# joybio/multiPrime

Measured on AMD Instinct MI355X. Metric: candidate x sequence coverage evals/s, higher is better.
Workload: dtype u32; 1 GPU; synthetic MSA 1048576 x 1000, k=18, v=1, 8 candidates/window, 950 windows, strict -c 2,3,-1 per GPU x 1 GPU(s) = BASELINE configs[3] itself (SURVEY 8d input 4; synthetic 1M x 1 kb; shape 1x1: row shards x window groups); rows_per_gpu=1048576, rows_total=1048576, cols=1000, k=18, variation=1, candidates_per_window=8, windows=950, parallelism=one GPU holds every row

## Files before the change

### multiprime_amd/csrc/evalslide.hip

```cpp
#include "common.hpp"
#include "bitslice.hpp"
#include "slidecore.hpp"
#include "evalslide.hpp"
#include "chainbody.hpp"

using namespace mp;

namespace {

typedef unsigned int u32x4 __attribute__((ext_vector_type(4)));
typedef unsigned int u32x2 __attribute__((ext_vector_type(2)));

struct SlideKernArgs {
    SlideArgs A;
    const uint32_t *cols32;
    const uint32_t *excl32;
    int nw32;
    unsigned long long *out;
    int wc, wc_pad;
    int max_items;
    int n_slide_blocks;
    EvalChainArgs chain;
    unsigned long long *clear;
    uint32_t n_clear;
    int patch_words;
    unsigned long long *stamps;
};

template <int GW>
struct DevEnv {
    const SlideKernArgs &K;
    __amdgpu_buffer_rsrc_t rs_cols, rs_excl;
    int voff, lane;
    uint32_t row_bytes;
    bool live;
    uint32_t *ring;
    uint32_t *tab;
    uint32_t itv;
    uint32_t live_mask;

    __device__ __forceinline__ DevEnv(const SlideKernArgs &k) : K(k) {}
    __device__ __forceinline__ void progress(int quarter) const {
#ifndef SLIDE_NO_PRIO
        if (quarter <= 0) __builtin_amdgcn_s_setprio(3);
        else if (quarter == 1) __builtin_amdgcn_s_setprio(2);
        else if (quarter == 2) __builtin_amdgcn_s_setprio(1);
        else __builtin_amdgcn_s_setprio(0);
#endif
    }
    __device__ __forceinline__ void stamp(int i) const {
        if (K.stamps && threadIdx.x == 0) K.stamps[(size_t)blockIdx.x * 8 + i] = wall_clock64();
    }
    __device__ __forceinline__ SlideBand uband(int b) const {
        const SlideBand *p = K.A.bands + b;
        SlideBand r;
        r.w0 = __builtin_amdgcn_readfirstlane(p->w0); r.n_win = __builtin_amdgcn_readfirstlane(p->n_win);
        r.item0 = __builtin_amdgcn_readfirstlane(p->item0); r.n_items = __builtin_amdgcn_readfirstlane(p->n_items);
        r.iter0 = __builtin_amdgcn_readfirstlane(p->iter0); r.pad = 0;
        return r;
    }
    __device__ __forceinline__ void load_iters(int idx) { itv = K.A.iters[(size_t)idx + (size_t)lane]; }
    __device__ __forceinline__ uint32_t iter_word(int j) const { return (uint32_t)__builtin_amdgcn_readlane((int)itv, j); }
    typedef const uint32_t __attribute__((address_space(4))) * ConstWords;
    struct Rec { uint32_t w[8], sm_lo, sm_hi, flags; ConstWords p; };
    __device__ __forceinline__ Rec load_rec(int item) const {
        Rec r;
        r.p = (ConstWords)(K.A.recs + (size_t)__builtin_amdgcn_readfirstlane(item) * kSlideRec);
#pragma unroll
        for (int q = 0; q < 8; q++) r.w[q] = r.p[q];
        r.sm_lo = r.p[24]; r.sm_hi = r.p[25]; r.flags = r.p[28];
        return r;
    }
    __device__ __forceinline__ uint32_t rec_word(const Rec &r, int q) const {
        return q < 8 ? r.w[q] : (q == 24 ? r.sm_lo : (q == 25 ? r.sm_hi : (q == 28 ? r.flags : r.p[q])));
    }
    __device__ __forceinline__ uint32_t rec_word_dyn(const Rec &r, int q) const { return r.p[q]; }
    template <int AUX = 0>
    __device__ __forceinline__ void load(__amdgpu_buffer_rsrc_t rs, int soff, uint32_t (&d)[GW]) const {
        if constexpr (GW == 4) {
            const u32x4 v = __builtin_amdgcn_raw_buffer_load_b128(rs, voff, soff, AUX);
            d[0] = v.x; d[1] = v.y; d[2] = v.z; d[3] = v.w;
        } else if constexpr (GW == 2) {
            const u32x2 v = __builtin_amdgcn_raw_buffer_load_b64(rs, voff, soff, AUX);
            d[0] = v.x; d[1] = v.y;
        } else {
            d[0] = __builtin_amdgcn_raw_buffer_load_b32(rs, voff, soff, AUX);
        }
    }
#ifndef SLIDE_EXP_ONE_ROW
#define SLIDE_EXP_ONE_ROW 0
#endif
#ifndef SLIDE_COL_AUX
#define SLIDE_COL_AUX 2
#endif
#ifndef SLIDE_EVT_AUX
#define SLIDE_EVT_AUX 0
#endif
    __device__ __forceinline__ void fetch(uint32_t row_off, uint32_t (&d)[GW]) const {
        load<SLIDE_COL_AUX>(rs_cols, SLIDE_EXP_ONE_ROW == 1 || SLIDE_EXP_ONE_ROW == 3 ? 0 : (int)row_off, d);
    }
    __device__ __forceinline__ void fetch_event(uint32_t row_off, uint32_t (&d)[GW]) const {
        load<SLIDE_EVT_AUX>(rs_cols, SLIDE_EXP_ONE_ROW == 1 || SLIDE_EXP_ONE_ROW == 2 ? 0 : (int)row_off, d);
    }
    __device__ __forceinline__ void valid_of(uint32_t row_off, uint32_t (&v)[GW]) const {
        load(rs_excl, (int)row_off, v);
#pragma unroll
        for (int i = 0; i < GW; i++) v[i] = bop<kSlAndNot>(live_mask, v[i], 0u);
    }
    __device__ __forceinline__ void ring_put(uint32_t *p, const uint32_t (&v)[GW]) const {
        if constexpr (GW == 4) *reinterpret_cast<u32x4 *>(p) = u32x4{v[0], v[1], v[2], v[3]};
        else if constexpr (GW == 2) *reinterpret_cast<u32x2 *>(p) = u32x2{v[0], v[1]};
        else p[0] = v[0];
    }
    __device__ __forceinline__ void ring_get(const uint32_t *p, uint32_t (&v)[GW]) const {
        if constexpr (GW == 4) { const u32x4 t = *reinterpret_cast<const u32x4 *>(p); v[0] = t.x; v[1] = t.y; v[2] = t.z; v[3] = t.w; }
        else if constexpr (GW == 2) { const u32x2 t = *reinterpret_cast<const u32x2 *>(p); v[0] = t.x; v[1] = t.y; }
        else v[0] = p[0];
    }
    __device__ __forceinline__ void ring_zero(int k) {
        uint32_t z[GW];
#pragma unroll
        for (int i = 0; i < GW; i++) z[i] = 0u;
        for (int s = 0; s < k; s++) ring_put(ring + s * (64 * GW), z);
    }
    __device__ __forceinline__ void ring_write(int slot, const uint32_t (&in)[GW]) { ring_put(ring + slot * (64 * GW), in); }
    __device__ __forceinline__ void ring_read(int slot, uint32_t (&o)[GW]) const { ring_get(ring + slot * (64 * GW), o); }
    __device__ __forceinline__ void commit(int idx, const uint32_t (&accPF)[8], const uint32_t (&accR)[4]) {
        uint32_t x0 = accPF[0], x1 = accPF[1], x2 = accPF[2], x3 = accPF[3], x4 = accPF[4], x5 = accPF[5], x6 = accPF[6], x7 = accPF[7];
        uint32_t x8 = accR[0], x9 = accR[1], x10 = accR[2], x11 = accR[3];
        asm volatile(
            "s_nop 1\n\t"
            "v_add_u32_dpp %0, %0, %0 row_ror:4 row_mask:0xf bank_mask:0x5\n\t"
            "v_add_u32_dpp %2, %2, %2 row_ror:4 row_mask:0xf bank_mask:0x5\n\t"
            "v_add_u32_dpp %4, %4, %4 row_ror:4 row_mask:0xf bank_mask:0x5\n\t"
            "v_add_u32_dpp %6, %6, %6 row_ror:4 row_mask:0xf bank_mask:0x5\n\t"
            "v_add_u32_dpp %8, %8, %8 row_ror:4 row_mask:0xf bank_mask:0x5\n\t"
            "v_add_u32_dpp %10, %10, %10 row_ror:4 row_mask:0xf bank_mask:0x5\n\t"
            "v_add_u32_dpp %0, %1, %1 row_ror:4 row_mask:0xf bank_mask:0xa\n\t"
            "v_add_u32_dpp %2, %3, %3 row_ror:4 row_mask:0xf bank_mask:0xa\n\t"
            "v_add_u32_dpp %4, %5, %5 row_ror:4 row_mask:0xf bank_mask:0xa\n\t"
            "v_add_u32_dpp %6, %7, %7 row_ror:4 row_mask:0xf bank_mask:0xa\n\t"
            "v_add_u32_dpp %8, %9, %9 row_ror:4 row_mask:0xf bank_mask:0xa\n\t"
            "v_add_u32_dpp %10, %11, %11 row_ror:4 row_mask:0xf bank_mask:0xa\n\t"
            "v_add_u32_dpp %0, %0, %0 row_ror:8 row_mask:0xf bank_mask:0x3\n\t"
            "v_add_u32_dpp %4, %4, %4 row_ror:8 row_mask:0xf bank_mask:0x3\n\t"
            "v_add_u32_dpp %8, %8, %8 row_ror:8 row_mask:0xf bank_mask:0x3\n\t"
            "v_add_u32_dpp %0, %2, %2 row_ror:8 row_mask:0xf bank_mask:0xc\n\t"
            "v_add_u32_dpp %4, %6, %6 row_ror:8 row_mask:0xf bank_mask:0xc\n\t"
            "v_add_u32_dpp %8, %10, %10 row_ror:8 row_mask:0xf bank_mask:0xc\n\t"
            "v_add_u32_dpp %0, %0, %0 quad_perm:[1,0,3,2] row_mask:0xf bank_mask:0xf\n\t"
            "v_add_u32_dpp %4, %4, %4 quad_perm:[1,0,3,2] row_mask:0xf bank_mask:0xf\n\t"
            "v_add_u32_dpp %8, %8, %8 quad_perm:[1,0,3,2] row_mask:0xf bank_mask:0xf\n\t"
            "v_add_u32_dpp %0, %0, %0 quad_perm:[2,3,0,1] row_mask:0xf bank_mask:0xf\n\t"
            "v_add_u32_dpp %4, %4, %4 quad_perm:[2,3,0,1] row_mask:0xf bank_mask:0xf\n\t"
            "v_add_u32_dpp %8, %8, %8 quad_perm:[2,3,0,1] row_mask:0xf bank_mask:0xf\n\t"
            "s_nop 1"
            : "+v"(x0), "+v"(x1), "+v"(x2), "+v"(x3), "+v"(x4), "+v"(x5), "+v"(x6), "+v"(x7), "+v"(x8), "+v"(x9), "+v"(x10), "+v"(x11));
        typedef unsigned int u32pair __attribute__((ext_vector_type(2)));
        const u32pair s01 = __builtin_amdgcn_permlane16_swap(x0, x4, false, false);
        const uint32_t a = s01.x + s01.y;
        const u32pair s22 = __builtin_amdgcn_permlane16_swap(x8, x8, false, false);
        const uint32_t b = s22.x + s22.y;
        const u32pair h = __builtin_amdgcn_permlane32_swap(a, b, false, false);
        const uint32_t tot = h.x + h.y;
        if (lane < 48 && (lane & 3) == 0) atomicAdd(&tab[idx * 12 + (lane >> 4) * 4 + ((lane >> 2) & 3)], tot);
    }
};

#ifndef SLIDE_MIN_WAVES
#define SLIDE_MIN_WAVES 1
#endif
template <int LV, int GW, bool FAST>
__global__ __launch_bounds__(kBlock, GW == 4 ? 1 : SLIDE_MIN_WAVES) void eval_slide_kernel(const SlideKernArgs K) {
    extern __shared__ __align__(16) uint32_t lds[];
    clear_counters(K.clear, K.n_clear, blockIdx.x, gridDim.x);
    if (K.stamps && threadIdx.x == 0) K.stamps[(size_t)blockIdx.x * 8] = wall_clock64();
    if ((int)blockIdx.x >= K.n_slide_blocks) {
        const unsigned pb = blockIdx.x - (unsigned)K.n_slide_blocks, wv = threadIdx.x >> 6;
#ifndef SLIDE_PATCH_PRIO
#define SLIDE_PATCH_PRIO 3
#endif
        __builtin_amdgcn_s_setprio(SLIDE_PATCH_PRIO);
        if (K.patch_words == 1) {
            const bool negative = (int)pb >= K.chain.patch.n_blocks;
            const unsigned unit = (pb - (negative ? (unsigned)K.chain.patch.n_blocks : 0u)) * (kBlock / 64) + wv;
            eval_patch_wave<LV>(K.chain, lds + wv * 12, lds + 64 + wv * (64 * kPatchEvents), unit, negative);
        } else {
            uint32_t(&s_part)[kBlock / 64][12] = *reinterpret_cast<uint32_t(*)[kBlock / 64][12]>(lds);
            eval_chain_block<LV, 8, 4>(K.chain, s_part, pb);
        }
        if (K.stamps && threadIdx.x == 0) K.stamps[(size_t)blockIdx.x * 8 + 7] = wall_clock64();
        return;
    }
    const int slice = (int)(blockIdx.x % (unsigned)K.wc_pad), band = (int)(blockIdx.x / (unsigned)K.wc_pad);
    if (slice >= K.wc) return;
    const int wv = (int)(threadIdx.x >> 6), lane = (int)(threadIdx.x & 63);
    const int ring_words = K.A.k * 64 * GW;
    uint32_t *tab = lds + (kBlock / 64) * ring_words;
    DevEnv<GW> env(K);
    env.lane = lane;
    env.ring = lds + wv * ring_words + lane * GW;
    env.tab = tab;
    env.itv = 0u;
    const int word0 = (slice * kBlock + (int)threadIdx.x) * GW;
    env.live = word0 < K.nw32;
    env.voff = env.live ? word0 * 4 : 0x7FFFFF00;
    env.live_mask = env.live ? 0xFFFFFFFFu : 0u;
    env.row_bytes = (uint32_t)K.nw32 * 4u;
    env.rs_cols = __builtin_amdgcn_make_buffer_rsrc(const_cast<uint32_t *>(K.cols32), 0, 0x7FFFFF00, 0x00020000);
    env.rs_excl = __builtin_amdgcn_make_buffer_rsrc(const_cast<uint32_t *>(K.excl32), 0, 0x7FFFFF00, 0x00020000);
    const SlideBand bd = env.uband(band);
    for (int i = (int)threadIdx.x; i < bd.n_items * 12; i += kBlock) tab[i] = 0u;
    __syncthreads();
    env.stamp(1);
    const bool wave_live = (slice * kBlock + wv * 64) * GW < K.nw32;
    if (wave_live) slide_band<LV, GW, true, false, FAST>(env, K.A, band);
    env.stamp(4);
    __syncthreads();
    env.stamp(5);
    int live_waves = 0;
    for (int w = 0; w < kBlock / 64; w++) live_waves += (slice * kBlock + w * 64) * GW < K.nw32 ? 1 : 0;
    const uint32_t rows = (uint32_t)live_waves * 64u * 32u * GW;
    const int n_entries = bd.n_items * 24;
    for (int i0 = (int)threadIdx.x; i0 < n_entries; i0 += 4 * kBlock) {
        int oc[4];
        uint32_t map[4];
#pragma unroll
        for (int u = 0; u < 4; u++) {
            const int i = i0 + u * kBlock, ic = i < n_entries ? i : (int)threadIdx.x;
            const uint32_t *rec = K.A.recs + (size_t)(bd.item0 + ic / 24) * kSlideRec;
            oc[u] = (int)rec[8 + (ic % 24) / 3];
            map[u] = rec[26];
        }
#pragma unroll
        for (int u = 0; u < 4; u++) {
            const int i = i0 + u * kBlock;
            if (i >= n_entries || oc[u] < 0) continue;
            const int item = i / 24, r = i % 24, t = r / 3, kind = r % 3;
            const int slot = (int)((map[u] >> (4 * t)) & 15u);
            const uint32_t *row = tab + item * 12;
            const uint32_t out1 = row[slot] & 0xFFFFu, outF = row[slot] >> 16, outR = (row[8 + (slot >> 1)] >> (16 * (slot & 1))) & 0xFFFFu;
            const uint32_t val = kind == 0 ? rows - out1 : out1 - (kind == 1 ? outF : outR);
            if (val) atomicAdd(&K.out[(size_t)oc[u] * 3 + kind], (unsigned long long)val);
        }
    }
    env.stamp(6);
}

typedef void (*SlideFn)(const SlideKernArgs);

}

namespace mp {

void free_slide(mp_ctx *c) {
    dev_free(c, &c->slide_bands, (size_t)c->slide_n_bands);
    dev_free(c, &c->slide_iters, c->slide_n_iters);
    dev_free(c, &c->slide_recs, (size_t)c->slide_items * kSlideRec);
    dev_free(c, &c->chain_rest, (size_t)c->n_rest);
    dev_free(c, &c->chain_slid, (size_t)c->slide_items);
    c->slide_items = c->slide_n_bands = c->slide_max_items = 0;
    c->slide_n_iters = 0;
    c->n_rest = c->rest_max_steps = 0;
}

int upload_eval_slide(mp_ctx *c, const std::vector<ChainItem> &chains, const std::vector<uint32_t> &events, const std::vector<int32_t> &cand_out) {
    free_slide(c);
    const char *se = getenv("MP_EVAL_SLIDE");
    if (chains.empty() || c->v > 3 || c->k <= c->v || (se ? atoi(se) != 1 : c->n_pad <= 262144)) return MP_OK;
    const int nw32 = c->n_pad / 32, n_cols = c->n_chunks * 32;
    if (((unsigned long long)n_cols * 4ull + 1ull) * (unsigned long long)nw32 * 4ull >= 0x7FFFFFFFull) return MP_OK;
    if ((unsigned long long)c->n_win * (unsigned long long)nw32 * 4ull >= 0x7FFFFFFFull) return MP_OK;
    int gw = 2;
    if (const char *e = getenv("MP_SLIDE_GW")) { const int g = atoi(e); if (g == 1 || g == 2 || g == 4) gw = g; }
    const int wc = (nw32 + kBlock * gw - 1) / (kBlock * gw), wc_pad = wc >= 8 ? (wc + 7) / 8 * 8 : wc;
    const int span = chains.back().win - chains.front().win + 1;
    std::vector<SlideChainIn> in(chains.size());
    for (size_t i = 0; i < chains.size(); i++) {
        const ChainItem &ch = chains[i];
        in[i] = SlideChainIn{ch.win, ch.cand0, ch.n_steps, ch.ev0, ch.n_ev, {ch.sym[0], ch.sym[1], ch.sym[2], ch.sym[3]}};
    }
    const size_t ring_bytes = (size_t)(kBlock / 64) * ((size_t)c->k * 64 * gw) * sizeof(uint32_t), lds_cu = 160 * 1024;
    int resident = (int)std::min<size_t>(4, std::max<size_t>(1, lds_cu / (ring_bytes + 1024)));
    if (gw == 4) resident = 1;
    SlidePlan P;
    for (;; resident--) {
        const int per_round = std::max(1, 256 * resident / std::max(1, wc_pad));
        int band = (span + per_round - 1) / per_round;
        for (int r = 2; band > 96; r++) band = (span + per_round * r - 1) / (per_round * r);
        band = std::max(8, band);
        if (const char *e = getenv("MP_SLIDE_BAND")) band = std::max(1, atoi(e));
        if (!build_slide_plan(in, events, cand_out, c->k, (uint32_t)c->sF, (uint32_t)c->sR, c->p0, n_cols, band, (uint32_t)nw32 * 4u, true, P)) return MP_OK;
        const size_t need = ring_bytes + (size_t)P.max_items_band * 12 * sizeof(uint32_t);
        if (resident <= 1 || need * (size_t)resident <= lds_cu) break;
    }
    P.iters.resize(P.iters.size() + 64, 0u);
    int rc;
    if ((rc = dev_alloc(c, &c->slide_bands, P.bands.size()))) return rc;
    c->slide_n_bands = (int)P.bands.size();
    if ((rc = dev_alloc(c, &c->slide_iters, P.iters.size()))) return rc;
    c->slide_n_iters = P.iters.size();
    c->slide_items = (int)P.item_of.size();
    if ((rc = dev_alloc(c, &c->slide_recs, P.recs.size()))) return rc;
    HIPCK(c, hipMemcpy(c->slide_bands, P.bands.data(), sizeof(SlideBand) * P.bands.size(), hipMemcpyHostToDevice));
    HIPCK(c, hipMemcpy(c->slide_iters, P.iters.data(), sizeof(uint32_t) * P.iters.size(), hipMemcpyHostToDevice));
    HIPCK(c, hipMemcpy(c->slide_recs, P.recs.data(), sizeof(uint32_t) * P.recs.size(), hipMemcpyHostToDevice));
    c->slide_max_items = P.max_items_band;
    c->slide_ns = P.ns; c->slide_spos = P.spos; c->slide_fmask = P.fmask; c->slide_rmask = P.rmask;
    c->slide_fast = slide_strict_lists(c->k, (uint32_t)c->sF, (uint32_t)c->sR, c->slide_fpos, c->slide_rpos);
    if (const char *e = getenv("MP_SLIDE_STRICT")) { if (atoi(e) == 0) c->slide_fast = false; }
    c->slide_gw = gw;
    {
        std::vector<ChainItem> slid;
        for (int32_t i : P.item_of) slid.push_back(chains[(size_t)i]);
        if ((rc = dev_alloc(c, &c->chain_slid, slid.size()))) return rc;
        HIPCK(c, hipMemcpy(c->chain_slid, slid.data(), sizeof(ChainItem) * slid.size(), hipMemcpyHostToDevice));
    }
    if (!P.rest.empty()) {
        std::vector<ChainItem> rest;
        for (int32_t i : P.rest) { rest.push_back(chains[(size_t)i]); c->rest_max_steps = std::max(c->rest_max_steps, (int)chains[(size_t)i].n_steps); }
        if ((rc = dev_alloc(c, &c->chain_rest, rest.size()))) return rc;
        c->n_rest = (int)rest.size();
        HIPCK(c, hipMemcpy(c->chain_rest, rest.data(), sizeof(ChainItem) * rest.size(), hipMemcpyHostToDevice));
    }
    return MP_OK;
}

int launch_eval_slide(mp_ctx *c, unsigned long long *device_out, const EvalChainArgs *patch, int patch_blocks, int patch_words,
                      unsigned long long *clear, uint32_t n_clear) {
#define SLIDE_ROW(LV, F) {eval_slide_kernel<LV, 1, F>, eval_slide_kernel<LV, 2, F>, eval_slide_kernel<LV, 4, F>}
    static const SlideFn fn[2][4][3] = {{SLIDE_ROW(1, false), SLIDE_ROW(2, false), SLIDE_ROW(3, false), SLIDE_ROW(4, false)},
                                        {SLIDE_ROW(1, true), SLIDE_ROW(2, true), SLIDE_ROW(3, true), SLIDE_ROW(4, true)}};
#undef SLIDE_ROW
    const int gw = c->slide_gw, gi = gw == 4 ? 2 : gw - 1;
    const int nw32 = c->n_pad / 32;
    SlideKernArgs K;
    K.A = SlideArgs{c->slide_bands, c->slide_iters, c->slide_recs, c->k, c->p0, c->slide_ns, c->slide_spos, c->slide_fmask, c->slide_rmask,
                    (uint32_t)nw32 * 4u, c->slide_fpos, c->slide_rpos};
    K.cols32 = reinterpret_cast<const uint32_t *>(c->cols);
    K.excl32 = reinterpret_cast<const uint32_t *>(c->excl);
    K.nw32 = nw32;
    K.out = device_out;
    K.wc = (nw32 + kBlock * gw - 1) / (kBlock * gw);
    K.wc_pad = K.wc >= 8 ? (K.wc + 7) / 8 * 8 : K.wc;
    K.max_items = c->slide_max_items;
    K.n_slide_blocks = c->slide_n_bands * K.wc_pad;
    if (patch) K.chain = *patch;
    else { memset(&K.chain, 0, sizeof K.chain); patch_blocks = 0; }
    K.chain.clear = nullptr; K.chain.n_clear = 0;
    K.clear = clear; K.n_clear = n_clear;
    K.patch_words = patch_words;
    K.stamps = nullptr;
    const char *stamp_file = getenv("MP_EXPERIMENT_STAMPS");
    const size_t n_stamp = ((size_t)K.n_slide_blocks + (size_t)patch_blocks) * 8;
    if (stamp_file) {
        HIPCK(c, hipMalloc(&K.stamps, n_stamp * sizeof(unsigned long long)));
        HIPCK(c, hipMemsetAsync(K.stamps, 0, n_stamp * sizeof(unsigned long long), c->stream));
    }
    size_t lds = ((size_t)(kBlock / 64) * ((size_t)c->k * 64 * gw) + (size_t)c->slide_max_items * 12) * sizeof(uint32_t);
    if (patch_blocks) lds = std::max(lds, (size_t)(64 + (kBlock / 64) * 64 * kPatchEvents) * sizeof(uint32_t));
    if (lds > 160 * 1024) return fail(c, MP_ERR_ARG, "sliding evaluation: a band needs %zu bytes of LDS", lds);
    SlideFn f = fn[c->slide_fast ? 1 : 0][c->v][gi];
    if (lds > 48 * 1024) HIPCK(c, hipFuncSetAttribute(reinterpret_cast<const void *>(f), hipFuncAttributeMaxDynamicSharedMemorySize, (int)lds));
    hipLaunchKernelGGL(f, dim3((unsigned)K.n_slide_blocks + (unsigned)patch_blocks), dim3(kBlock), lds, c->stream, K);
    HIPCK(c, hipGetLastError());
    if (stamp_file) {
        std::vector<unsigned long long> h(n_stamp + 2);
        HIPCK(c, hipStreamSynchronize(c->stream));
        HIPCK(c, hipMemcpy(h.data() + 2, K.stamps, n_stamp * sizeof(unsigned long long), hipMemcpyDeviceToHost));
        HIPCK(c, hipFree(K.stamps));
        h[0] = (unsigned long long)K.n_slide_blocks; h[1] = (unsigned long long)patch_blocks;
        if (FILE *fo = fopen(stamp_file, "wb")) { fwrite(h.data(), sizeof(unsigned long long), h.size(), fo); fclose(fo); }
    }
    return MP_OK;
}

}
```

### multiprime_amd/csrc/slidecore.hpp

```cpp
#pragma once

#include <cstdint>

#include "slideplan.hpp"

#if defined(__HIPCC__)
#define SLIDE_HD __host__ __device__ __forceinline__
#else
#define SLIDE_HD inline
#endif

#ifndef SLIDE_UNLIKELY
#define SLIDE_UNLIKELY(x) __builtin_expect(!!(x), 0)
#endif

namespace mp {

template <int LUT>
SLIDE_HD uint32_t bop(uint32_t a, uint32_t b, uint32_t c) {
#if defined(__HIP_DEVICE_COMPILE__)
    return __builtin_amdgcn_bitop3_b32(a, b, c, LUT);
#else
    uint32_t r = 0;
    if (LUT & 0x01) r |= ~a & ~b & ~c;
    if (LUT & 0x02) r |= ~a & ~b & c;
    if (LUT & 0x04) r |= ~a & b & ~c;
    if (LUT & 0x08) r |= ~a & b & c;
    if (LUT & 0x10) r |= a & ~b & ~c;
    if (LUT & 0x20) r |= a & ~b & c;
    if (LUT & 0x40) r |= a & b & ~c;
    if (LUT & 0x80) r |= a & b & c;
    return r;
#endif
}
constexpr int slide_lut(bool (*f)(bool, bool, bool)) {
    int t = 0;
    for (int i = 0; i < 8; i++)
        if (f((i >> 2) & 1, (i >> 1) & 1, i & 1)) t |= 1 << i;
    return t;
}
constexpr int kSlXor3 = slide_lut([](bool a, bool b, bool c) { return (a != b) != c; });
constexpr int kSlMaj = slide_lut([](bool a, bool b, bool c) { return (a && b) || (a && c) || (b && c); });
constexpr int kSlProp = slide_lut([](bool p, bool ci, bool dir) { return p && (ci == dir); });
constexpr int kSlBorrow = slide_lut([](bool ci, bool s, bool br) { return (!ci && s) || (!ci && br) || (s && br); });
constexpr int kSlAndNot = slide_lut([](bool a, bool b, bool) { return a && !b; });
constexpr int kSlOr3 = slide_lut([](bool a, bool b, bool c) { return a || b || c; });
constexpr int kSlOrAnd = slide_lut([](bool a, bool b, bool c) { return a || (b && c); });
constexpr int kSlOrAndNot = slide_lut([](bool a, bool b, bool c) { return a || (b && !c); });
constexpr int kSlAndNotNot = slide_lut([](bool a, bool b, bool c) { return a && !b && !c; });
constexpr int kSlOrNot = slide_lut([](bool a, bool b, bool) { return a || !b; });
constexpr int kSlOrOrNot = slide_lut([](bool a, bool b, bool c) { return a || b || !c; });
constexpr int kSlXorAndNot = slide_lut([](bool a, bool b, bool c) { return a != (b && !c); });

SLIDE_HD int slide_popc(uint32_t x) {
#if defined(__HIP_DEVICE_COMPILE__)
    return __popc(x);
#else
    return __builtin_popcount(x);
#endif
}

SLIDE_HD void slide_pin(uint32_t &x) {
#if defined(__HIP_DEVICE_COMPILE__)
    asm volatile("" : "+v"(x));
#else
    (void)x;
#endif
}

struct SlideCount { uint32_t b0, b1, b2, b3, b4; };
SLIDE_HD void slide_updown(SlideCount &c, uint32_t x, uint32_t dir) {
    uint32_t p = x;
    uint32_t n = c.b0 ^ p; p = bop<kSlProp>(p, c.b0, dir); c.b0 = n;
    n = c.b1 ^ p; p = bop<kSlProp>(p, c.b1, dir); c.b1 = n;
    n = c.b2 ^ p; p = bop<kSlProp>(p, c.b2, dir); c.b2 = n;
    n = c.b3 ^ p; p = bop<kSlProp>(p, c.b3, dir); c.b3 = n;
    c.b4 ^= p;
}

struct SlideArgs {
    const SlideBand *bands;
    const uint32_t *iters;
    const uint32_t *recs;
    int k, p0, ns;
    uint32_t spos, fmask, rmask;
    uint32_t row_scale;
    uint32_t fpos, rpos;
};

inline bool slide_strict_lists(int k, uint32_t sF, uint32_t sR, uint32_t &fpos, uint32_t &rpos) {
    fpos = rpos = 0u;
    uint32_t nf = 0, nr = 0;
    for (int j = 0; j < k && j < 32; j++) {
        if ((sF >> j) & 1u) { if (nf == 3) return false; fpos |= (uint32_t)j << (5 * nf++); }
        if ((sR >> j) & 1u) { if (nr == 3) return false; rpos |= (uint32_t)j << (5 * nr++); }
    }
    fpos |= nf << 15; rpos |= nr << 15;
    return true;
}

template <int GW>
struct SlideFetch {
    uint32_t d[kSlideKept + 1][GW];
    uint32_t valid[GW];
};

template <int GW, bool USE_VALID, class Env>
SLIDE_HD void slide_request(Env &env, const typename Env::Rec &rec, SlideFetch<GW> &F) {
    if (USE_VALID) env.valid_of(env.rec_word(rec, 29), F.valid);
#pragma unroll
    for (int s = 1; s <= kSlideKept; s++) env.fetch_event(env.rec_word(rec, s), F.d[s]);
}

template <int LV, int GW, bool SIMPLE, bool USE_VALID, bool NO_EXTRA, bool FAST, class Env>
SLIDE_HD void slide_item(Env &env, const SlideArgs &A, const typename Env::Rec &rec, uint32_t hdr, const SlideCount (&cnt)[GW],
                         const uint32_t (&sv)[kSlideStrict][GW], const SlideFetch<GW> &F, uint32_t (&accPF)[8], uint32_t (&accR)[4]) {
    const int n_extra = (int)((hdr >> 8) & 15u);
    const uint32_t flags = env.rec_word(rec, 28);
    SlideCount c0[GW];
    uint32_t sub[kSlideKept + 1];
#pragma unroll
    for (int s = 1; s <= kSlideKept; s++) sub[s] = SIMPLE ? 0xFFFFFFFFu : (uint32_t)((int32_t)(flags << (15 - s)) >> 31);
#pragma unroll
    for (int i = 0; i < GW; i++) {
        uint32_t e[kSlideKept + 1];
#pragma unroll
        for (int s = 1; s <= kSlideKept; s++) e[s] = SIMPLE ? F.d[s][i] : (F.d[s][i] & sub[s]);
        const uint32_t sa = bop<kSlXor3>(e[1], e[2], e[3]), ca = bop<kSlMaj>(e[1], e[2], e[3]);
        const uint32_t sb = bop<kSlXor3>(e[4], e[5], e[6]), cb = bop<kSlMaj>(e[4], e[5], e[6]);
        const uint32_t s0 = bop<kSlXor3>(sa, sb, e[7]), cc = bop<kSlMaj>(sa, sb, e[7]);
        const uint32_t s1 = bop<kSlXor3>(ca, cb, cc), s2 = bop<kSlMaj>(ca, cb, cc);
        const SlideCount c = cnt[i];
        SlideCount r;
        r.b0 = c.b0 ^ s0;
        uint32_t br = bop<kSlAndNot>(s0, c.b0, 0u);
        r.b1 = bop<kSlXor3>(c.b1, s1, br); br = bop<kSlBorrow>(c.b1, s1, br);
        r.b2 = bop<kSlXor3>(c.b2, s2, br); br = bop<kSlBorrow>(c.b2, s2, br);
        r.b3 = c.b3 ^ br; br = bop<kSlAndNot>(br, c.b3, 0u);
        r.b4 = c.b4 ^ br;
        c0[i] = r;
    }
    if (!NO_EXTRA && n_extra) {
        const uint32_t row0 = env.rec_word(rec, 30);
#pragma unroll 1
        for (int x = 0; x < n_extra; x++) {
            const uint32_t ex = env.rec_word_dyn(rec, 16 + x);
            uint32_t pl[GW];
            env.fetch(row0 + (ex & 127u) * A.row_scale, pl);
            const uint32_t up = (ex & kSlSub) ? 0u : 0xFFFFFFFFu;
#pragma unroll
            for (int i = 0; i < GW; i++) slide_updown(c0[i], pl[i], up);
        }
    }
    uint32_t T[4][GW], DF[GW], DR[GW];
    const uint32_t sm_lo = env.rec_word(rec, 24), sm_hi = env.rec_word(rec, 25);
#pragma unroll
    for (int i = 0; i < GW; i++) DF[i] = DR[i] = 0u;
    uint32_t cF0[GW], cF1[GW], cR0[GW], cR1[GW];
    if (FAST) {
        static_assert(!FAST || SIMPLE, "the two-bit strict counts take back SUB planes only");
#pragma unroll
        for (int i = 0; i < GW; i++) { cF0[i] = sv[0][i]; cF1[i] = sv[1][i]; cR0[i] = sv[2][i]; cR1[i] = sv[3][i]; }
#pragma unroll
        for (int s = 1; s <= kSlideKept; s++) {
            if (SLIDE_UNLIKELY(((flags >> s) & 0x101u) != 0u)) {
                if ((flags >> s) & 1u) {
#pragma unroll
                    for (int i = 0; i < GW; i++) { cF1[i] = bop<kSlXorAndNot>(cF1[i], F.d[s][i], cF0[i]); cF0[i] ^= F.d[s][i]; }
                }
                if ((flags >> (8 + s)) & 1u) {
#pragma unroll
                    for (int i = 0; i < GW; i++) { cR1[i] = bop<kSlXorAndNot>(cR1[i], F.d[s][i], cR0[i]); cR0[i] ^= F.d[s][i]; }
                }
            }
        }
    }
#pragma unroll
    for (int q = 0; q < kSlideStrict; q++) {
        if (FAST) break;
        if (q >= 4 && A.ns <= 4) break;
        const uint32_t sm = ((q < 4 ? sm_lo : sm_hi) >> (8 * (q & 3))) & 255u;
        const uint32_t nfF = ~(uint32_t)((int32_t)(A.fmask << (31 - q)) >> 31), nfR = ~(uint32_t)((int32_t)(A.rmask << (31 - q)) >> 31);
        if (SLIDE_UNLIKELY(sm != 0u)) {
            uint32_t x[GW];
#pragma unroll
            for (int i = 0; i < GW; i++) x[i] = 0u;
#pragma unroll
            for (int s = 1; s <= kSlideKept; s++) {
                const uint32_t m = (uint32_t)((int32_t)(sm << (31 - s)) >> 31);
#pragma unroll
                for (int i = 0; i < GW; i++) x[i] = bop<kSlOrAnd>(x[i], F.d[s][i], m);
            }
#pragma unroll
            for (int i = 0; i < GW; i++) {
                DF[i] = bop<kSlOrAndNot>(DF[i], sv[q][i], x[i] | nfF);
                DR[i] = bop<kSlOrAndNot>(DR[i], sv[q][i], x[i] | nfR);
            }
        } else {
#pragma unroll
            for (int i = 0; i < GW; i++) {
                DF[i] = bop<kSlOrAndNot>(DF[i], sv[q][i], nfF);
                DR[i] = bop<kSlOrAndNot>(DR[i], sv[q][i], nfR);
            }
        }
    }
#pragma unroll
    for (int i = 0; i < GW; i++) {
        const SlideCount c = c0[i];
        const uint32_t hi = bop<kSlOr3>(c.b2, c.b3, c.b4);
        const uint32_t t1 = bop<kSlOr3>(c.b0, c.b1, hi), t2 = c.b1 | hi, t3 = bop<kSlOrAnd>(hi, c.b1, c.b0);
        const uint32_t far = LV == 1 ? t1 : (LV == 2 ? t2 : (LV == 3 ? t3 : hi));
        T[0][i] = USE_VALID ? bop<kSlOrNot>(t1, F.valid[i], 0u) : t1;
        T[1][i] = t2; T[2][i] = t3; T[3][i] = hi;
        if (FAST && !USE_VALID) {
            DF[i] = bop<kSlOr3>(cF0[i], cF1[i], far);
            DR[i] = bop<kSlOr3>(cR0[i], cR1[i], far);
        } else {
            if (FAST) { DF[i] = cF0[i] | cF1[i]; DR[i] = cR0[i] | cR1[i]; }
            DF[i] = USE_VALID ? bop<kSlOrOrNot>(DF[i], far, F.valid[i]) : (DF[i] | far);
            DR[i] = USE_VALID ? bop<kSlOrOrNot>(DR[i], far, F.valid[i]) : (DR[i] | far);
        }
    }
#pragma unroll
    for (int s = 0; s < 8; s++) {
        if (s > 0) {
#ifndef SLIDE_WALK_BRANCH
#define SLIDE_WALK_BRANCH 2
#endif
            if (SLIDE_WALK_BRANCH == 2) {
#pragma unroll
                for (int i = 0; i < GW; i++) {
                    const uint32_t d = F.d[s][i];
                    if (LV == 1) { DF[i] |= d; DR[i] |= d; }
                    else {
                        DF[i] = bop<kSlOrAnd>(DF[i], d, T[LV >= 2 ? LV - 2 : 0][i]);
                        DR[i] = bop<kSlOrAnd>(DR[i], d, T[LV >= 2 ? LV - 2 : 0][i]);
                    }
                }
                if (LV >= 2 && SLIDE_UNLIKELY(((flags >> s) & 0x101u) != 0u)) {
                    const uint32_t mF = (uint32_t)((int32_t)(flags << (31 - s)) >> 31), mR = (uint32_t)((int32_t)(flags << (23 - s)) >> 31);
#pragma unroll
                    for (int i = 0; i < GW; i++) {
                        DF[i] = bop<kSlOrAnd>(DF[i], F.d[s][i], mF);
                        DR[i] = bop<kSlOrAnd>(DR[i], F.d[s][i], mR);
                    }
                }
            } else if (LV >= 2 && (!SLIDE_WALK_BRANCH || ((flags >> s) & 0x101u))) {
                const uint32_t mF = (uint32_t)((int32_t)(flags << (31 - s)) >> 31), mR = (uint32_t)((int32_t)(flags << (23 - s)) >> 31);
#pragma unroll
                for (int i = 0; i < GW; i++) {
                    const uint32_t d = F.d[s][i], t = T[LV >= 2 ? LV - 2 : 0][i];
                    DF[i] = bop<kSlOrAnd>(DF[i], d, t | mF);
                    DR[i] = bop<kSlOrAnd>(DR[i], d, t | mR);
                }
            } else {
#pragma unroll
                for (int i = 0; i < GW; i++) {
                    const uint32_t d = F.d[s][i];
                    if (LV == 1) { DF[i] |= d; DR[i] |= d; }
                    else {
                        DF[i] = bop<kSlOrAnd>(DF[i], d, T[LV >= 2 ? LV - 2 : 0][i]);
                        DR[i] = bop<kSlOrAnd>(DR[i], d, T[LV >= 2 ? LV - 2 : 0][i]);
                    }
                }
            }
#pragma unroll
            for (int i = 0; i < GW; i++) {
                const uint32_t d = F.d[s][i];
                if (LV >= 4) T[2][i] = bop<kSlOrAnd>(T[2][i], T[1][i], d);
                if (LV >= 3) T[1][i] = bop<kSlOrAnd>(T[1][i], T[0][i], d);
                T[0][i] |= d;
            }
        }
        uint32_t nP = 0, nF = 0, nR = 0;
#pragma unroll
        for (int i = 0; i < GW; i++) {
            nP += (uint32_t)slide_popc(T[0][i]);
            nF += (uint32_t)slide_popc(DF[i]);
            nR += (uint32_t)slide_popc(DR[i]);
        }
        accPF[s] = nP | (nF << 16);
        if (s & 1) accR[s >> 1] |= nR << 16;
        else accR[s >> 1] = nR;
        if (SLIDE_WALK_BRANCH) { slide_pin(accPF[s]); slide_pin(accR[s >> 1]); }
    }
}

template <int N, int GW, class Env>
SLIDE_HD void slide_warm_chunk(Env &env, SlideCount (&cnt)[GW], int &slot, int j) {
    uint32_t w[N][GW];
#pragma unroll
    for (int u = 0; u < N; u++) env.fetch(env.iter_word(2 * (j + u)), w[u]);
#pragma unroll
    for (int u = 0; u < N; u++) {
        uint32_t bn[GW];
#pragma unroll
        for (int i = 0; i < GW; i++) {
            bn[i] = ~w[u][i];
            slide_updown(cnt[i], bn[i], bn[i]);
        }
        env.ring_write(slot, bn);
        slot++;
    }
}

template <int LV, int GW, bool ONLY_SIMPLE, bool USE_VALID, bool FAST = false, class Env>
SLIDE_HD void slide_band(Env &env, const SlideArgs &A, int band_index) {
    static_assert(LV >= 1 && LV <= 4 && GW >= 1 && GW <= 4, "counter levels / words per lane");
    static_assert(!FAST || ONLY_SIMPLE, "FAST strict counts: simple items only");
    const SlideBand bd = env.uband(band_index);
    const int k = A.k;
    SlideCount cnt[GW];
#pragma unroll
    for (int i = 0; i < GW; i++) cnt[i] = SlideCount{0u, 0u, 0u, 0u, 0u};
    env.ring_zero(k);
    int slot = 0;
    const int n_iter = bd.n_win + k - 1;
    const int last_item = bd.item0 + bd.n_items - 1;
    typename Env::Rec rec0 = env.load_rec(bd.item0), rec1 = env.load_rec(bd.item0 + 1 <= last_item ? bd.item0 + 1 : last_item);
    SlideFetch<GW> F0, F1;
    slide_request<GW, USE_VALID>(env, rec0, F0);
    int done = 0;
    env.load_iters(bd.iter0);
    env.stamp(2);
    int j0 = 0;
    {
        const int n_warm = k - 1 < n_iter ? k - 1 : n_iter;
        while (n_warm - j0 >= 16) { slide_warm_chunk<16, GW>(env, cnt, slot, j0); j0 += 16; }
        if (n_warm - j0 >= 8) { slide_warm_chunk<8, GW>(env, cnt, slot, j0); j0 += 8; }
        if (n_warm - j0 >= 4) { slide_warm_chunk<4, GW>(env, cnt, slot, j0); j0 += 4; }
        if (n_warm - j0 >= 2) { slide_warm_chunk<2, GW>(env, cnt, slot, j0); j0 += 2; }
    }
    env.stamp(3);
    uint32_t bA[GW], bB[GW];
    env.fetch(env.iter_word(2 * j0), bA);
    env.fetch(env.iter_word(n_iter > j0 + 1 ? 2 * j0 + 2 : 2 * j0), bB);

    auto item = [&](typename Env::Rec &rec_cur, typename Env::Rec &rec_other, const SlideFetch<GW> &F_cur, SlideFetch<GW> &F_other,
                    const uint32_t (&sv)[kSlideStrict][GW]) __attribute__((always_inline)) {
        const int after = bd.item0 + done + 2;
        const typename Env::Rec rec = rec_cur;
        rec_cur = env.load_rec(after <= last_item ? after : last_item);
        slide_request<GW, USE_VALID>(env, rec_other, F_other);
        const uint32_t hdr = env.rec_word(rec, 0);
        uint32_t accPF[8], accR[4];
        if (ONLY_SIMPLE || (hdr & kSlSimple)) slide_item<LV, GW, true, USE_VALID, ONLY_SIMPLE, FAST>(env, A, rec, hdr, cnt, sv, F_cur, accPF, accR);
        else slide_item<LV, GW, false, USE_VALID, false, false>(env, A, rec, hdr, cnt, sv, F_cur, accPF, accR);
        env.commit(done, accPF, accR);
        done++;
    };
    auto iteration = [&](uint32_t (&b)[GW], uint32_t (&bo)[GW], uint32_t (&bo_next)[GW], int j) __attribute__((always_inline)) {
        const uint32_t it1 = env.iter_word(2 * j + 1);
        uint32_t bn[GW];
#pragma unroll
        for (int i = 0; i < GW; i++) bn[i] = ~b[i];
        env.fetch(env.iter_word(2 * j + 4), b);
#pragma unroll
        for (int i = 0; i < GW; i++) slide_updown(cnt[i], bn[i] ^ bo[i], bn[i]);
        env.ring_write(slot, bn);
        const int slot_now = slot;
        slot = slot + 1 == k ? 0 : slot + 1;
        env.ring_read(slot, bo_next);
        const int n_items = (int)(it1 >> 24);
        if (n_items == 0) return;
        uint32_t sv[kSlideStrict][GW];
        if (FAST) {
            uint32_t p[2][3][GW];
#pragma unroll
            for (int side = 0; side < 2; side++) {
                const uint32_t pos = side ? A.rpos : A.fpos;
                const int n = (int)(pos >> 15);
#pragma unroll
                for (int q = 0; q < 3; q++) {
                    if (SLIDE_UNLIKELY(q >= n)) {
#pragma unroll
                        for (int i = 0; i < GW; i++) p[side][q][i] = 0u;
                    } else {
                        int s = slot_now + 1 + (int)((pos >> (5 * q)) & 31u);
                        if (s >= k) s -= k;
                        env.ring_read(s, p[side][q]);
                    }
                }
            }
#pragma unroll
            for (int side = 0; side < 2; side++)
#pragma unroll
                for (int i = 0; i < GW; i++) {
                    sv[2 * side][i] = bop<kSlXor3>(p[side][0][i], p[side][1][i], p[side][2][i]);
                    sv[2 * side + 1][i] = bop<kSlMaj>(p[side][0][i], p[side][1][i], p[side][2][i]);
                }
        }
#pragma unroll
        for (int q = 0; q < kSlideStrict; q++) {
            if (FAST) break;
            if (q < 4 || A.ns > 4) {
                int s = slot_now + 1 + (int)((A.spos >> (5 * q)) & 31u);
                if (s >= k) s -= k;
                env.ring_read(s, sv[q]);
            } else {
#pragma unroll
                for (int i = 0; i < GW; i++) sv[q][i] = 0u;
            }
        }
        int ii = 0;
        if (done & 1) { item(rec1, rec0, F1, F0, sv); ii = 1; }
#pragma unroll 1
        for (; ii + 1 < n_items; ii += 2) {
            item(rec0, rec1, F0, F1, sv);
            item(rec1, rec0, F1, F0, sv);
        }
        if (ii < n_items) item(rec0, rec1, F0, F1, sv);
    };
#ifndef SLIDE_PRIO_MIN_WIN
#define SLIDE_PRIO_MIN_WIN 32
#endif
    const int quarter_len = bd.n_win < SLIDE_PRIO_MIN_WIN ? 1 << 20 : ((bd.n_win + 3) / 4 > 2 ? (bd.n_win + 3) / 4 : 2);
    int quarter = 0, next_quarter = k - 1 + quarter_len;
    env.progress(0);
    uint32_t boA[GW], boB[GW];
    env.ring_read(slot, boA);
#pragma unroll 1
    for (int base = 0; base < n_iter; base += 30) {
        if (base) env.load_iters(bd.iter0 + 2 * base);
        const int n_here = n_iter - base < 30 ? n_iter - base : 30;
        int j = base ? 0 : j0;
#pragma unroll 1
        for (; j + 1 < n_here; j += 2) {
            if (base + j >= next_quarter) { env.progress(++quarter); next_quarter += quarter_len; }
            iteration(bA, boA, boB, j);
            iteration(bB, boB, boA, j + 1);
        }
        if (j < n_here) iteration(bA, boA, boB, j);
    }
    env.progress(3);
}

}
```

Before: 59320 billion evals/s.

## Dedupe strict ring reads via shape-specialized loops and incremental byte offsets

Strict forward and reverse position lists are merged on the host into a distinct set plus a shape code (shared, forward-only, reverse-only). The kernel dispatches to a template specialized on that shape, so each distinct ring slot is read once per iteration instead of up to six times. Ring addressing switches from slot indices with modulo and multiply to byte offsets that advance incrementally. The cost is more template instantiations and code size, plus extra registers for the per-position offsets.

```diff
diff --git a/multiprime_amd/csrc/evalslide.hip b/multiprime_amd/csrc/evalslide.hip
--- a/multiprime_amd/csrc/evalslide.hip
+++ b/multiprime_amd/csrc/evalslide.hip
@@ -123,8 +123,10 @@
         for (int i = 0; i < GW; i++) z[i] = 0u;
         for (int s = 0; s < k; s++) ring_put(ring + s * (64 * GW), z);
     }
-    __device__ __forceinline__ void ring_write(int slot, const uint32_t (&in)[GW]) { ring_put(ring + slot * (64 * GW), in); }
-    __device__ __forceinline__ void ring_read(int slot, uint32_t (&o)[GW]) const { ring_get(ring + slot * (64 * GW), o); }
+    __device__ __forceinline__ uint32_t ring_step() const { return 64u * GW * (uint32_t)sizeof(uint32_t); }
+    __device__ __forceinline__ uint32_t *ring_at(uint32_t off) const { return reinterpret_cast<uint32_t *>(reinterpret_cast<char *>(ring) + off); }
+    __device__ __forceinline__ void ring_write(uint32_t off, const uint32_t (&in)[GW]) { ring_put(ring_at(off), in); }
+    __device__ __forceinline__ void ring_read(uint32_t off, uint32_t (&o)[GW]) const { ring_get(ring_at(off), o); }
     __device__ __forceinline__ void commit(int idx, const uint32_t (&accPF)[8], const uint32_t (&accR)[4]) {
         uint32_t x0 = accPF[0], x1 = accPF[1], x2 = accPF[2], x3 = accPF[3], x4 = accPF[4], x5 = accPF[5], x6 = accPF[6], x7 = accPF[7];
         uint32_t x8 = accR[0], x9 = accR[1], x10 = accR[2], x11 = accR[3];
@@ -336,7 +338,8 @@
     const int nw32 = c->n_pad / 32;
     SlideKernArgs K;
     K.A = SlideArgs{c->slide_bands, c->slide_iters, c->slide_recs, c->k, c->p0, c->slide_ns, c->slide_spos, c->slide_fmask, c->slide_rmask,
-                    (uint32_t)nw32 * 4u, c->slide_fpos, c->slide_rpos};
+                    (uint32_t)nw32 * 4u, c->slide_fpos, c->slide_rpos, 0u, 0u};
+    if (c->slide_fast) slide_strict_distinct(c->slide_fpos, c->slide_rpos, K.A.dpos, K.A.dshape);
     K.cols32 = reinterpret_cast<const uint32_t *>(c->cols);
     K.excl32 = reinterpret_cast<const uint32_t *>(c->excl);
     K.nw32 = nw32;
diff --git a/multiprime_amd/csrc/slidecore.hpp b/multiprime_amd/csrc/slidecore.hpp
--- a/multiprime_amd/csrc/slidecore.hpp
+++ b/multiprime_amd/csrc/slidecore.hpp
@@ -86,6 +86,7 @@
     uint32_t spos, fmask, rmask;
     uint32_t row_scale;
     uint32_t fpos, rpos;
+    uint32_t dpos, dshape;
 };
 
 inline bool slide_strict_lists(int k, uint32_t sF, uint32_t sR, uint32_t &fpos, uint32_t &rpos) {
@@ -98,6 +99,25 @@
     fpos |= nf << 15; rpos |= nr << 15;
     return true;
 }
+
+inline void slide_strict_distinct(uint32_t fpos, uint32_t rpos, uint32_t &dpos, uint32_t &dshape) {
+    const int nf = (int)(fpos >> 15), nr = (int)(rpos >> 15);
+    uint32_t fm = 0, rm = 0;
+    for (int q = 0; q < nf; q++) fm |= 1u << ((fpos >> (5 * q)) & 31u);
+    for (int q = 0; q < nr; q++) rm |= 1u << ((rpos >> (5 * q)) & 31u);
+    const uint32_t sets[3] = {fm & rm, fm & ~rm, rm & ~fm};
+    int n = 0, cnt[3] = {0, 0, 0};
+    dpos = 0u;
+    for (int c = 0; c < 3; c++)
+        for (int j = 0; j < 32; j++)
+            if ((sets[c] >> j) & 1u) { dpos |= (uint32_t)j << (5 * n++); cnt[c]++; }
+    dshape = (uint32_t)cnt[0] | ((uint32_t)cnt[1] << 2) | ((uint32_t)cnt[2] << 4);
+}
+constexpr uint32_t slide_shape_code(int nb, int nfo, int nro) { return (uint32_t)nb | ((uint32_t)nfo << 2) | ((uint32_t)nro << 4); }
+constexpr uint32_t kSlShapeDefault = slide_shape_code(1, 1, 2);
+
+template <int NB_, int NFO_, int NRO_, bool MASKED_>
+struct SlideShape { static constexpr int NB = NB_, NFO = NFO_, NRO = NRO_, ND = NB_ + NFO_ + NRO_; static constexpr bool MASKED = MASKED_; };
 
 template <int GW>
 struct SlideFetch {
@@ -287,7 +307,7 @@
 }
 
 template <int N, int GW, class Env>
-SLIDE_HD void slide_warm_chunk(Env &env, SlideCount (&cnt)[GW], int &slot, int j) {
+SLIDE_HD void slide_warm_chunk(Env &env, SlideCount (&cnt)[GW], uint32_t &cur, int j) {
     uint32_t w[N][GW];
 #pragma unroll
     for (int u = 0; u < N; u++) env.fetch(env.iter_word(2 * (j + u)), w[u]);
@@ -299,8 +319,8 @@
             bn[i] = ~w[u][i];
             slide_updown(cnt[i], bn[i], bn[i]);
         }
-        env.ring_write(slot, bn);
-        slot++;
+        env.ring_write(cur, bn);
+        cur += env.ring_step();
     }
 }
 
@@ -314,7 +334,8 @@
 #pragma unroll
     for (int i = 0; i < GW; i++) cnt[i] = SlideCount{0u, 0u, 0u, 0u, 0u};
     env.ring_zero(k);
-    int slot = 0;
+    const uint32_t ring_step = env.ring_step(), ring_end = (uint32_t)k * ring_step;
+    uint32_t cur = 0u;
     const int n_iter = bd.n_win + k - 1;
     const int last_item = bd.item0 + bd.n_items - 1;
     typename Env::Rec rec0 = env.load_rec(bd.item0), rec1 = env.load_rec(bd.item0 + 1 <= last_item ? bd.item0 + 1 : last_item);
@@ -326,10 +347,10 @@
     int j0 = 0;
     {
         const int n_warm = k - 1 < n_iter ? k - 1 : n_iter;
-        while (n_warm - j0 >= 16) { slide_warm_chunk<16, GW>(env, cnt, slot, j0); j0 += 16; }
-        if (n_warm - j0 >= 8) { slide_warm_chunk<8, GW>(env, cnt, slot, j0); j0 += 8; }
-        if (n_warm - j0 >= 4) { slide_warm_chunk<4, GW>(env, cnt, slot, j0); j0 += 4; }
-        if (n_warm - j0 >= 2) { slide_warm_chunk<2, GW>(env, cnt, slot, j0); j0 += 2; }
+        while (n_warm - j0 >= 16) { slide_warm_chunk<16, GW>(env, cnt, cur, j0); j0 += 16; }
+        if (n_warm - j0 >= 8) { slide_warm_chunk<8, GW>(env, cnt, cur, j0); j0 += 8; }
+        if (n_warm - j0 >= 4) { slide_warm_chunk<4, GW>(env, cnt, cur, j0); j0 += 4; }
+        if (n_warm - j0 >= 2) { slide_warm_chunk<2, GW>(env, cnt, cur, j0); j0 += 2; }
     }
     env.stamp(3);
     uint32_t bA[GW], bB[GW];
@@ -349,88 +370,123 @@
         env.commit(done, accPF, accR);
         done++;
     };
-    auto iteration = [&](uint32_t (&b)[GW], uint32_t (&bo)[GW], uint32_t (&bo_next)[GW], int j) __attribute__((always_inline)) {
-        const uint32_t it1 = env.iter_word(2 * j + 1);
-        uint32_t bn[GW];
-#pragma unroll
-        for (int i = 0; i < GW; i++) bn[i] = ~b[i];
-        env.fetch(env.iter_word(2 * j + 4), b);
-#pragma unroll
-        for (int i = 0; i < GW; i++) slide_updown(cnt[i], bn[i] ^ bo[i], bn[i]);
-        env.ring_write(slot, bn);
-        const int slot_now = slot;
-        slot = slot + 1 == k ? 0 : slot + 1;
-        env.ring_read(slot, bo_next);
-        const int n_items = (int)(it1 >> 24);
-        if (n_items == 0) return;
-        uint32_t sv[kSlideStrict][GW];
-        if (FAST) {
-            uint32_t p[2][3][GW];
-#pragma unroll
-            for (int side = 0; side < 2; side++) {
-                const uint32_t pos = side ? A.rpos : A.fpos;
-                const int n = (int)(pos >> 15);
-#pragma unroll
-                for (int q = 0; q < 3; q++) {
-                    if (SLIDE_UNLIKELY(q >= n)) {
-#pragma unroll
-                        for (int i = 0; i < GW; i++) p[side][q][i] = 0u;
-                    } else {
-                        int s = slot_now + 1 + (int)((pos >> (5 * q)) & 31u);
-                        if (s >= k) s -= k;
-                        env.ring_read(s, p[side][q]);
-                    }
-                }
-            }
-#pragma unroll
-            for (int side = 0; side < 2; side++)
-#pragma unroll
-                for (int i = 0; i < GW; i++) {
-                    sv[2 * side][i] = bop<kSlXor3>(p[side][0][i], p[side][1][i], p[side][2][i]);
-                    sv[2 * side + 1][i] = bop<kSlMaj>(p[side][0][i], p[side][1][i], p[side][2][i]);
-                }
-        }
-#pragma unroll
-        for (int q = 0; q < kSlideStrict; q++) {
-            if (FAST) break;
-            if (q < 4 || A.ns > 4) {
-                int s = slot_now + 1 + (int)((A.spos >> (5 * q)) & 31u);
-                if (s >= k) s -= k;
-                env.ring_read(s, sv[q]);
-            } else {
-#pragma unroll
-                for (int i = 0; i < GW; i++) sv[q][i] = 0u;
-            }
-        }
-        int ii = 0;
-        if (done & 1) { item(rec1, rec0, F1, F0, sv); ii = 1; }
-#pragma unroll 1
-        for (; ii + 1 < n_items; ii += 2) {
-            item(rec0, rec1, F0, F1, sv);
-            item(rec1, rec0, F1, F0, sv);
-        }
-        if (ii < n_items) item(rec0, rec1, F0, F1, sv);
-    };
 #ifndef SLIDE_PRIO_MIN_WIN
 #define SLIDE_PRIO_MIN_WIN 32
 #endif
     const int quarter_len = bd.n_win < SLIDE_PRIO_MIN_WIN ? 1 << 20 : ((bd.n_win + 3) / 4 > 2 ? (bd.n_win + 3) / 4 : 2);
-    int quarter = 0, next_quarter = k - 1 + quarter_len;
-    env.progress(0);
-    uint32_t boA[GW], boB[GW];
-    env.ring_read(slot, boA);
+    auto run = [&](auto shape) __attribute__((always_inline)) {
+        typedef decltype(shape) Shape;
+        constexpr int NS = Shape::ND;
+        uint32_t so[NS > 0 ? NS : 1], sm[NS > 0 ? NS : 1];
+#pragma unroll
+        for (int q = 0; q < NS; q++) {
+            uint32_t pos, present = 1u;
+            if (!FAST) pos = (A.spos >> (5 * q)) & 31u;
+            else if (!Shape::MASKED) pos = (A.dpos >> (5 * q)) & 31u;
+            else {
+                const uint32_t list = q < 3 ? A.fpos : A.rpos;
+                const int qq = q < 3 ? q : q - 3;
+                present = qq < (int)(list >> 15) ? 1u : 0u;
+                pos = present ? (list >> (5 * qq)) & 31u : 0u;
+            }
+            so[q] = (((uint32_t)j0 + pos) % (uint32_t)k) * ring_step;
+            sm[q] = present ? 0xFFFFFFFFu : 0u;
+        }
+        auto iteration = [&](uint32_t (&b)[GW], uint32_t (&bo)[GW], uint32_t (&bo_next)[GW], int j) __attribute__((always_inline)) {
+            const uint32_t it1 = env.iter_word(2 * j + 1);
+            uint32_t bn[GW];
+#pragma unroll
+            for (int i = 0; i < GW; i++) bn[i] = ~b[i];
+            env.fetch(env.iter_word(2 * j + 4), b);
+#pragma unroll
+            for (int i = 0; i < GW; i++) slide_updown(cnt[i], bn[i] ^ bo[i], bn[i]);
+            env.ring_write(cur, bn);
+            cur += ring_step;
+            if (cur == ring_end) cur = 0u;
+            env.ring_read(cur, bo_next);
+#pragma unroll
+            for (int q = 0; q < NS; q++) {
+                so[q] += ring_step;
+                if (so[q] == ring_end) so[q] = 0u;
+            }
+            const int n_items = (int)(it1 >> 24);
+            if (n_items == 0) return;
+            uint32_t sv[kSlideStrict][GW];
+            if (FAST) {
+                uint32_t d[NS > 0 ? NS : 1][GW];
+#pragma unroll
+                for (int q = 0; q < NS; q++) {
+                    env.ring_read(so[q], d[q]);
+                    if (Shape::MASKED) {
+#pragma unroll
+                        for (int i = 0; i < GW; i++) d[q][i] &= sm[q];
+                    }
+                }
+                constexpr int NF = Shape::NB + Shape::NFO, NR = Shape::NB + Shape::NRO;
+                static_assert(NF <= 3 && NR <= 3, "at most three strict positions per side");
+#pragma unroll
+                for (int i = 0; i < GW; i++) {
+                    uint32_t f[3] = {0u, 0u, 0u}, r[3] = {0u, 0u, 0u};
+#pragma unroll
+                    for (int q = 0; q < NF; q++) f[q] = d[q][i];
+#pragma unroll
+                    for (int q = 0; q < NR; q++) r[q] = d[q < Shape::NB ? q : q + Shape::NFO][i];
+                    sv[0][i] = NF == 3 ? bop<kSlXor3>(f[0], f[1], f[2]) : (f[0] ^ f[1]);
+                    sv[1][i] = NF == 3 ? bop<kSlMaj>(f[0], f[1], f[2]) : (f[0] & f[1]);
+                    sv[2][i] = NR == 3 ? bop<kSlXor3>(r[0], r[1], r[2]) : (r[0] ^ r[1]);
+                    sv[3][i] = NR == 3 ? bop<kSlMaj>(r[0], r[1], r[2]) : (r[0] & r[1]);
+                }
+            }
+#pragma unroll
+            for (int q = 0; q < kSlideStrict; q++) {
+                if (FAST) break;
+                if (q < NS) {
+                    env.ring_read(so[q], sv[q]);
+                } else {
+#pragma unroll
+                    for (int i = 0; i < GW; i++) sv[q][i] = 0u;
+                }
+            }
+            int ii = 0;
+            if (done & 1) { item(rec1, rec0, F1, F0, sv); ii = 1; }
 #pragma unroll 1
-    for (int base = 0; base < n_iter; base += 30) {
-        if (base) env.load_iters(bd.iter0 + 2 * base);
-        const int n_here = n_iter - base < 30 ? n_iter - base : 30;
-        int j = base ? 0 : j0;
+            for (; ii + 1 < n_items; ii += 2) {
+                item(rec0, rec1, F0, F1, sv);
+                item(rec1, rec0, F1, F0, sv);
+            }
+            if (ii < n_items) item(rec0, rec1, F0, F1, sv);
+        };
+        int quarter = 0, next_quarter = k - 1 + quarter_len;
+        env.progress(0);
+        uint32_t boA[GW], boB[GW];
+        env.ring_read(cur, boA);
 #pragma unroll 1
-        for (; j + 1 < n_here; j += 2) {
-            if (base + j >= next_quarter) { env.progress(++quarter); next_quarter += quarter_len; }
-            iteration(bA, boA, boB, j);
-            iteration(bB, boB, boA, j + 1);
-        }
-        if (j < n_here) iteration(bA, boA, boB, j);
+        for (int base = 0; base < n_iter; base += 30) {
+            if (base) env.load_iters(bd.iter0 + 2 * base);
+            const int n_here = n_iter - base < 30 ? n_iter - base : 30;
+            int j = base ? 0 : j0;
+#pragma unroll 1
+            for (; j + 1 < n_here; j += 2) {
+                if (base + j >= next_quarter) { env.progress(++quarter); next_quarter += quarter_len; }
+                iteration(bA, boA, boB, j);
+                iteration(bB, boB, boA, j + 1);
+            }
+            if (j < n_here) iteration(bA, boA, boB, j);
+        }
+    };
+    if constexpr (!FAST) {
+        if (A.ns > 4) run(SlideShape<0, 3, 3, false>());
+        else run(SlideShape<0, 2, 2, false>());
+    } else {
+        switch (A.dshape) {
+            case kSlShapeDefault: run(SlideShape<1, 1, 2, false>()); break;
+            case slide_shape_code(0, 0, 0): run(SlideShape<0, 0, 0, false>()); break;
+            case slide_shape_code(1, 0, 0): run(SlideShape<1, 0, 0, false>()); break;
+            case slide_shape_code(0, 1, 1): run(SlideShape<0, 1, 1, false>()); break;
+            case slide_shape_code(0, 2, 2): run(SlideShape<0, 2, 2, false>()); break;
+            case slide_shape_code(0, 3, 3): run(SlideShape<0, 3, 3, false>()); break;
+            default: run(SlideShape<0, 3, 3, true>()); break;
+        }
     }
     env.progress(3);
 }
```

Result: faster. 62080 billion evals/s (median of 6 runs) (+4.7%).
